# alanqrwang/nwhead

Measured on AMD Instinct MI355X. Metric: query-predictions/sec, higher is better.
Workload: dtype f32; 1 GPU; K3 predict('full'): B=256 queries/step vs bank N=50000 d=512 C=200, bank sharded 1-way, 26 query batches coalesced per launch; B=256, N_support=50000, d=512, C=200, parallelism=support-shard x1

## Files before the change

### nwhead_amd/csrc/fused_f16p12.h

```cpp
#pragma once
#include "fused_f16p.h"

namespace nw {
namespace {

struct P12 : PipeCfg<128, 256, 8, 4, 3> {
    static constexpr int RS = BS / 16, QB = BQP / (16 * NCW);
    static_assert(LDS_BYTES <= 160 * 1024, "LDS of one CU");
};

template <int KIND, bool CAND = false>
__device__ __forceinline__ void epilogue_p12(f32x4 (&acc)[P12::QB][P12::RS], const float* hdr, int nrun, int2 bnd,
                                             float scale, float* __restrict__ ws_m,
                                             float* __restrict__ ws_den, float* __restrict__ ws_num, int B, int N,
                                             int q0, int s0, int st, int wave, int lane, int n_stiles, int k
#ifdef NW_DIAG_FUSED
                                             , unsigned long long (&diag_)[8], unsigned long long& last_
#endif
                                             ) {
    using P = P12;
    constexpr int RS = P::RS, QB = P::QB, BS = P::BS;
    constexpr bool NEED_NORM = (KIND != NW_SCORE_DOT);
    typedef float f32x2 __attribute__((ext_vector_type(2)));
    const float* sn2 = hdr;
    const float* ssc = hdr + P::NH;
    const int* runid = reinterpret_cast<const int*>(hdr + 2 * P::NH);
    const float* qn2 = hdr + 3 * P::NH;
    const float* qsc_s = qn2 + P::BQP;
    const int i = lane & 15, g = lane >> 4;
    using SF = ScoreFactors<KIND>;
    float Cq[QB], Bq[QB];
#pragma unroll
    for (int j = 0; j < QB; ++j) {
        const int qrow = 16 * (QB * wave + j) + i;
        SF::query(NEED_NORM ? qn2[qrow] : 0.f, qsc_s[qrow], scale, Cq[j], Bq[j]);
    }
    NW_PSTAMP(1);
    float sc[QB][RS][4];
#pragma unroll
    for (int r = 0; r < RS; ++r) {
        const float4 n4 = NEED_NORM ? *reinterpret_cast<const float4*>(sn2 + 16 * r + 4 * g) : make_float4(0.f, 0.f, 0.f, 0.f);
        const float4 s4 = *reinterpret_cast<const float4*>(ssc + 16 * r + 4 * g);
        float4 K4, B4;
        SF::support(n4.x, s4.x, K4.x, B4.x);
        SF::support(n4.y, s4.y, K4.y, B4.y);
        SF::support(n4.z, s4.z, K4.z, B4.z);
        SF::support(n4.w, s4.w, K4.w, B4.w);
        float4 B4r = B4;
        asm volatile("" : "+v"(B4r.x), "+v"(B4r.y), "+v"(B4r.z), "+v"(B4r.w));
#pragma unroll
        for (int j = 0; j < QB; ++j) {
            const f32x2 cq = {Cq[j], Cq[j]}, bq = {Bq[j], Bq[j]};
            const float4 Bj = (j == 0) ? B4 : B4r;
            const f32x2 d01 = __builtin_elementwise_fma(f32x2{acc[j][r][0], acc[j][r][1]}, f32x2{K4.x, K4.y} * cq,
                                                        f32x2{Bj.x, Bj.y} + bq);
            const f32x2 d23 = __builtin_elementwise_fma(f32x2{acc[j][r][2], acc[j][r][3]}, f32x2{K4.z, K4.w} * cq,
                                                        f32x2{Bj.z, Bj.w} + bq);
            sc[j][r][0] = SF::finish_abs(d01.x);
            sc[j][r][1] = SF::finish_abs(d01.y);
            sc[j][r][2] = SF::finish_abs(d23.x);
            sc[j][r][3] = SF::finish_abs(d23.y);
            asm volatile("" : "+v"(sc[j][r][0]), "+v"(sc[j][r][1]), "+v"(sc[j][r][2]), "+v"(sc[j][r][3]));
        }
        __builtin_amdgcn_sched_barrier(0);
    }
    NW_PSTAMP(2);
    if constexpr (CAND) {
        int ln = lane;
        asm volatile("" : "+v"(ln));
        const int ci = ln & 15, cg = ln >> 4;
#pragma unroll
        for (int j = 0; j < QB; ++j) {
            float u[RS][4];
#pragma unroll
            for (int r = 0; r < RS; ++r)
#pragma unroll
                for (int e = 0; e < 4; ++e) u[r][e] = SF::DIST ? -sc[j][r][e] : sc[j][r][e];
            tile_candidates<RS>(u, reinterpret_cast<unsigned*>(ws_m), reinterpret_cast<int*>(ws_den), B, N,
                                q0 + 16 * (QB * wave + j) + ci, s0, cg, st, n_stiles, k);
            __builtin_amdgcn_sched_barrier(0);
        }
        return;
    }
    constexpr float WORST = SF::DIST ? INFINITY : -INFINITY;
    if (s0 + BS > N) {
        const int lim = N - s0 - 4 * g;
#pragma unroll
        for (int j = 0; j < QB; ++j)
#pragma unroll
            for (int r = 0; r < RS; ++r)
#pragma unroll
                for (int e = 0; e < 4; ++e)
                    if (16 * r + e >= lim) sc[j][r][e] = WORST;
    }
    auto best = [](float a, float b) { return SF::DIST ? fminf(a, b) : fmaxf(a, b); };
    auto best3 = [&](float a, float b, float c) { return best(best(a, b), c); };
    static_assert(RS == 8, "chain k takes the 16-row blocks k and k + 4");
    float ext[QB];
#pragma unroll
    for (int j = 0; j < QB; ++j) {
        float mx[4];
#pragma unroll
        for (int k = 0; k < 4; ++k) mx[k] = best3(sc[j][k][0], sc[j][k][1], sc[j][k][2]);
#pragma unroll
        for (int k = 0; k < 4; ++k) mx[k] = best3(mx[k], sc[j][k][3], sc[j][k + 4][0]);
#pragma unroll
        for (int k = 0; k < 4; ++k) mx[k] = best3(mx[k], sc[j][k + 4][1], sc[j][k + 4][2]);
#pragma unroll
        for (int k = 0; k < 4; ++k) mx[k] = best(mx[k], sc[j][k + 4][3]);
        ext[j] = best(best3(mx[0], mx[1], mx[2]), mx[3]);
    }
    group4_each(ext, best);
    float mloc[QB], dloc[QB], s0v[QB], s1v[QB] = {0.f, 0.f}, s2v[QB] = {0.f, 0.f};
#pragma unroll
    for (int j = 0; j < QB; ++j) {
        mloc[j] = SF::DIST ? -ext[j] : ext[j];
#pragma unroll
        for (int r = 0; r < RS; ++r)
#pragma unroll
            for (int e = 0; e < 4; ++e)
                sc[j][r][e] = __builtin_amdgcn_exp2f(SF::DIST ? ext[j] - sc[j][r][e] : sc[j][r][e] - ext[j]);
    }
    NW_PSTAMP(3);
    auto add = [](float a, float b) { return a + b; };
    if (nrun <= 3) {
        float S0[QB][2] = {{0.f, 0.f}, {0.f, 0.f}}, S1[QB][2] = {{0.f, 0.f}, {0.f, 0.f}}, S2[QB][2] = {{0.f, 0.f}, {0.f, 0.f}};
        if (nrun == 1) {
#pragma unroll
            for (int r = 0; r < RS; ++r)
#pragma unroll
                for (int j = 0; j < QB; ++j) S0[j][r & 1] += (sc[j][r][0] + sc[j][r][1]) + (sc[j][r][2] + sc[j][r][3]);
        } else {
            const int b1 = bnd.x, b2 = (nrun == 3) ? bnd.y : BS;
            const float L1 = (float)(b1 - 4 * g);
            const float M2 = 1.f - (float)(b2 - 4 * g);
#pragma unroll
            for (int r = 0; r < RS; ++r) {
                const int lo = 16 * r, hi = 16 * r + 16;
                const bool in0 = hi <= b1, in2 = lo >= b2, in1 = lo >= b1 && hi <= b2;
#pragma unroll
                for (int j = 0; j < QB; ++j) {
                    const float quad = (sc[j][r][0] + sc[j][r][1]) + (sc[j][r][2] + sc[j][r][3]);
                    S0[j][r & 1] = __builtin_fmaf(in0 ? 1.f : 0.f, quad, S0[j][r & 1]);
                    S1[j][r & 1] = __builtin_fmaf(in1 ? 1.f : 0.f, quad, S1[j][r & 1]);
                    S2[j][r & 1] = __builtin_fmaf(in2 ? 1.f : 0.f, quad, S2[j][r & 1]);
                }
                if (!(in0 || in1 || in2)) {
#pragma unroll
                    for (int e = 0; e < 4; ++e) {
                        const float c = (float)(16 * r + e);
                        const float w1 = __builtin_amdgcn_fmed3f(L1 - c, 0.f, 1.f);
                        const float u2 = __builtin_amdgcn_fmed3f(c + M2, 0.f, 1.f);
#pragma unroll
                        for (int j = 0; j < QB; ++j) {
                            const float ev = sc[j][r][e];
                            S0[j][e & 1] = __builtin_fmaf(w1, ev, S0[j][e & 1]);
                            S2[j][e & 1] = __builtin_fmaf(u2, ev, S2[j][e & 1]);
                            S1[j][e & 1] = __builtin_fmaf((1.f - w1) - u2, ev, S1[j][e & 1]);
                        }
                    }
                }
            }
        }
        if (nrun == 1) {
            float v[QB] = {S0[0][0] + S0[0][1], S0[1][0] + S0[1][1]};
            group4_each(v, add);
            s0v[0] = v[0], s0v[1] = v[1];
        } else if (nrun == 2) {
            float v[2 * QB] = {S0[0][0] + S0[0][1], S0[1][0] + S0[1][1], S1[0][0] + S1[0][1], S1[1][0] + S1[1][1]};
            group4_each(v, add);
            s0v[0] = v[0], s0v[1] = v[1], s1v[0] = v[2], s1v[1] = v[3];
        } else {
            float v[3 * QB] = {S0[0][0] + S0[0][1], S0[1][0] + S0[1][1], S1[0][0] + S1[0][1],
                               S1[1][0] + S1[1][1], S2[0][0] + S2[0][1], S2[1][0] + S2[1][1]};
            group4_each(v, add);
            s0v[0] = v[0], s0v[1] = v[1], s1v[0] = v[2], s1v[1] = v[3], s2v[0] = v[4], s2v[1] = v[5];
        }
#pragma unroll
        for (int j = 0; j < QB; ++j) dloc[j] = (s0v[j] + s1v[j]) + s2v[j];
    } else {
#pragma unroll
        for (int j = 0; j < QB; ++j) {
            float dl[4] = {0.f, 0.f, 0.f, 0.f};
#pragma unroll
            for (int r = 0; r < RS; ++r) dl[r & 3] += (sc[j][r][0] + sc[j][r][1]) + (sc[j][r][2] + sc[j][r][3]);
            dloc[j] = (dl[0] + dl[1]) + (dl[2] + dl[3]);
        }
        group4_each(dloc, add);
#pragma unroll
        for (int j = 0; j < QB; ++j) {
            const int b = q0 + 16 * (QB * wave + j) + i;
            for (int run_base = 0; run_base < nrun; run_base += 16) {
                f32x4 Pm = {0.f, 0.f, 0.f, 0.f};
                const int want = run_base + i;
#pragma unroll
                for (int r = 0; r < RS; ++r) {
                    const int4 rid = *reinterpret_cast<const int4*>(runid + 16 * r + 4 * g);
                    Pm = __builtin_amdgcn_mfma_f32_16x16x4f32(rid.x == want ? 1.f : 0.f, sc[j][r][0], Pm, 0, 0, 0);
                    Pm = __builtin_amdgcn_mfma_f32_16x16x4f32(rid.y == want ? 1.f : 0.f, sc[j][r][1], Pm, 0, 0, 0);
                    Pm = __builtin_amdgcn_mfma_f32_16x16x4f32(rid.z == want ? 1.f : 0.f, sc[j][r][2], Pm, 0, 0, 0);
                    Pm = __builtin_amdgcn_mfma_f32_16x16x4f32(rid.w == want ? 1.f : 0.f, sc[j][r][3], Pm, 0, 0, 0);
                }
                if (b < B) {
#pragma unroll
                    for (int jj = 0; jj < 4; ++jj) {
                        const int run = run_base + 4 * g + jj;
                        if (run < nrun) ws_num[((size_t)st * BS + run) * B + b] = Pm[jj];
                    }
                }
            }
        }
    }
    NW_PSTAMP(4);
    static_assert(QB == 2, "lane groups 0 / 1 carry query blocks 0 / 1, groups 2 / 3 the same blocks of the next array");
    int ln = lane;
    asm volatile("" : "+v"(ln));
    const int b = q0 + 16 * QB * wave + (ln & 31);
    const bool blk1 = ln & 16, arr1 = ln & 32;
    const size_t tb = (size_t)st * B + b, nb = (size_t)st * BS * B + b;
    if (b < B) {
        const float mv = blk1 ? mloc[1] : mloc[0], dv = blk1 ? dloc[1] : dloc[0];
        (arr1 ? ws_den : ws_m)[tb] = arr1 ? dv : mv;
        if (nrun <= 3) {
            const float n0 = blk1 ? s0v[1] : s0v[0], n1 = blk1 ? s1v[1] : s1v[0], n2 = blk1 ? s2v[1] : s2v[0];
            if (!arr1 || nrun >= 2) ws_num[nb + (arr1 ? B : 0)] = arr1 ? n1 : n0;
            if (!arr1 && nrun == 3) ws_num[nb + 2 * (size_t)B] = n2;
        }
    }
    NW_PSTAMP(5);
}

template <int KIND, bool HALF = false, bool CAND = false>
__global__ __launch_bounds__(P12::THREADS, 3) void nw_fused_f16p_kernel_w12(
    const float* __restrict__ q, const float* __restrict__ s, const float* __restrict__ s_norm2,
    const float* __restrict__ s_scale, const float* __restrict__ q_norm2, const float* __restrict__ q_scale,
    const float* __restrict__ logit_scale, const int* __restrict__ ws_runid, const int* __restrict__ ws_nrun,
    const int* __restrict__ ws_bnd, float* __restrict__ ws_m, float* __restrict__ ws_den, float* __restrict__ ws_num, int B,
    int N, int d, int n_stiles, int n_qtiles, int qg, int k) {
    static_assert(!CAND || HALF, "the candidate form exists for half-precision rows only");
    using P = P12;
    constexpr int RS = P::RS, QB = P::QB, BS = P::BS, BQP = P::BQP, NB = P::NB;
    extern __shared__ __attribute__((aligned(16))) char smem[];
    float* hdr0 = reinterpret_cast<float*>(smem);
    float4* stage = reinterpret_cast<float4*>(smem + P::HDR_BYTES);

    const int tid = threadIdx.x, lane = tid & 63;
    const int wave = __builtin_amdgcn_readfirstlane(tid >> 6);
    const int nk = d / BK;
    const PersistentTiles tiles(blockIdx.x, gridDim.x, n_stiles, n_qtiles, qg);
    const int cu = tiles.cu, n_cu = tiles.n_cu, n_local = tiles.n_local;

    if (wave >= P::NCW) {
        persistent_loader<P, !CAND>(tiles, wave - P::NCW, lane, hdr0, stage, q, s, s_norm2, s_scale, q_norm2, q_scale, ws_runid, B, N,
                             d);
    } else {
        const int i = lane & 15, g = lane >> 4;
        const int rsw = (i >> 1) & 7;
        const int sh = g ^ rsw, sl = (4 + g) ^ rsw;
        const int qoff = (16 * QB * wave + i) * ROW_F4, soff = (BQP + i) * ROW_F4;
        struct QF { float4 bh[QB], bl[QB]; };
        struct SW { float4 al[2], ah[2]; };
        constexpr int NW_ = RS / 2;
        auto rd_q = [&](QF& f, const float4* S) {
#pragma unroll
            for (int j = 0; j < QB; ++j) {
                f.bh[j] = S[qoff + 16 * j * ROW_F4 + sh];
                f.bl[j] = S[qoff + 16 * j * ROW_F4 + sl];
            }
        };
        auto rd_w = [&](SW& w, const float4* S, int p) {
#pragma unroll
            for (int x = 0; x < 2; ++x) {
                w.al[x] = S[soff + 16 * (2 * p + x) * ROW_F4 + sl];
                w.ah[x] = S[soff + 16 * (2 * p + x) * ROW_F4 + sh];
            }
        };
        auto mm = [](const float4& a, const float4& b, f32x4 c) {
            return __builtin_amdgcn_mfma_f32_16x16x32_f16(__builtin_bit_cast(half8, a), __builtin_bit_cast(half8, b), c, 0, 0, 0);
        };
        auto pin = []() { __builtin_amdgcn_sched_barrier(0); };
        f32x4 acc[QB][RS];
        auto mm_w = [&](const SW& w, const QF& f, int p) {
            if constexpr (HALF) {
#pragma unroll
                for (int x = 0; x < 2; ++x)
#pragma unroll
                    for (int j = 0; j < QB; ++j) acc[j][2 * p + x] = mm(w.ah[x], f.bh[j], acc[j][2 * p + x]);
#pragma unroll
                for (int x = 0; x < 2; ++x)
#pragma unroll
                    for (int j = 0; j < QB; ++j) acc[j][2 * p + x] = mm(w.al[x], f.bl[j], acc[j][2 * p + x]);
            } else {
#pragma unroll
                for (int x = 0; x < 2; ++x)
#pragma unroll
                    for (int j = 0; j < QB; ++j) acc[j][2 * p + x] = mm(w.al[x], f.bh[j], acc[j][2 * p + x]);
#pragma unroll
                for (int x = 0; x < 2; ++x)
#pragma unroll
                    for (int j = 0; j < QB; ++j) acc[j][2 * p + x] = mm(w.ah[x], f.bl[j], acc[j][2 * p + x]);
#pragma unroll
                for (int x = 0; x < 2; ++x)
#pragma unroll
                    for (int j = 0; j < QB; ++j) acc[j][2 * p + x] = mm(w.ah[x], f.bh[j], acc[j][2 * p + x]);
            }
            __builtin_amdgcn_sched_barrier(0);
        };
        SW wa, wb;
        auto run_stage = [&](const QF& fp, QF& fc, int slot, auto first) {
            constexpr bool FIRST = decltype(first)::value;
#ifdef NW_ABL_NORD
            constexpr bool RD = FIRST;
#else
            constexpr bool RD = true;
#endif
            const float4* S = stage + slot * P::TILE_F4;
            if (RD) { rd_q(fc, S); rd_w(wa, S, 0); }
            pin();
            if (!FIRST) mm_w(wb, fp, NW_ - 1);
#pragma unroll
            for (int p = 0; p + 1 < NW_; ++p) {
                if (RD) rd_w((p & 1) ? wa : wb, S, p + 1);
                pin();
                mm_w((p & 1) ? wb : wa, fc, p);
            }
            static_assert(NW_ % 2 == 0, "the last pair of a stage sits in wb");
            tile_barrier();
        };
        using Yes = std::integral_constant<bool, true>;
        using No = std::integral_constant<bool, false>;

        float scale = 1.f;
        if (KIND == NW_SCORE_CLIP)
            scale = __builtin_bit_cast(float, __builtin_amdgcn_readfirstlane(__builtin_bit_cast(int, expf(*logit_scale))));
        tile_barrier();
        int gi = 0;
        int par = 0;
        auto next_slot = [&]() {
            const int b = gi;
            gi = (gi + 1 == NB) ? 0 : gi + 1;
            return b;
        };
#ifdef NW_DIAG_FUSED
        unsigned long long diag_[8] = {0, 0, 0, 0, 0, 0, 0, 0}, last_ = __builtin_amdgcn_s_memtime();
        const unsigned long long first_ = last_, first_rt_ = __builtin_amdgcn_s_memrealtime();
#endif
        for (int T = cu; T < n_local; T += n_cu) {
            int qt, st;
            tiles.decode(T, qt, st);
            const int q0 = qt * BQP, s0 = st * BS;
            int nrun = 0;
            int2 bnd = {0, 0};
            if constexpr (!CAND) {
                nrun = ws_nrun[st];
                bnd = *reinterpret_cast<const int2*>(ws_bnd + 2 * (size_t)st);
            }
#pragma unroll
            for (int j = 0; j < QB; ++j)
#pragma unroll
                for (int r = 0; r < RS; ++r) acc[j][r] = f32x4{0.f, 0.f, 0.f, 0.f};
            QF f0, f1;
#ifdef NW_ABL_NORD
            rd_q(f1, stage + gi * P::TILE_F4);
#endif
            run_stage(f1, f0, next_slot(), Yes{});
            int kt = 1;
            for (; kt + 1 < nk; kt += 2) {
                run_stage(f0, f1, next_slot(), No{});
                run_stage(f1, f0, next_slot(), No{});
            }
            if (kt < nk) {
                run_stage(f0, f1, next_slot(), No{});
                mm_w(wb, f1, NW_ - 1);
            } else {
                mm_w(wb, f0, NW_ - 1);
            }
            NW_PSTAMP(0);
#ifndef NW_ABL_NOEPI
            epilogue_p12<KIND, CAND>(acc, hdr0 + par * P::HDR_F, nrun, bnd, scale, ws_m, ws_den, ws_num, B, N, q0, s0, st, wave,
                                     lane, n_stiles, k
#ifdef NW_DIAG_FUSED
                                     , diag_, last_
#endif
                                     );
#else
            keep_acc_alive(acc, ws_m, nrun, bnd);
#endif
            par = (par + 1 == P::NHB) ? 0 : par + 1;
            NW_PSTAMP(6);
        }
#ifdef NW_DIAG_FUSED
        diag_write_out(diag_, last_, first_, first_rt_);
#endif
    }
}

}
}
```

Before: 7.653 million query-predictions/s.

## Interleave LDS fragment reads with individual MFMAs and use incrementing LDS pointers

Replaces the grouped read-then-MFMA pattern in the compute waves with a per-MFMA schedule. Each LDS read for the next query and support fragments is issued between single MFMA instructions, separated by sched_barrier pins, so that LDS latency hides behind matrix work, including across the stage boundary. LDS addresses are now kept as raw address-space-3 offsets that advance per ring slot, instead of being recomputed from the slot index. It also adds optional head-timing diagnostics, and the rigid manual schedule may lose to the compiler's own scheduling or raise register pressure.

```diff
diff --git a/nwhead_amd/csrc/fused_f16p12.h b/nwhead_amd/csrc/fused_f16p12.h
--- a/nwhead_amd/csrc/fused_f16p12.h
+++ b/nwhead_amd/csrc/fused_f16p12.h
@@ -261,52 +261,70 @@
         struct QF { float4 bh[QB], bl[QB]; };
         struct SW { float4 al[2], ah[2]; };
         constexpr int NW_ = RS / 2;
-        auto rd_q = [&](QF& f, const float4* S) {
-#pragma unroll
-            for (int j = 0; j < QB; ++j) {
-                f.bh[j] = S[qoff + 16 * j * ROW_F4 + sh];
-                f.bl[j] = S[qoff + 16 * j * ROW_F4 + sl];
-            }
-        };
-        auto rd_w = [&](SW& w, const float4* S, int p) {
-#pragma unroll
-            for (int x = 0; x < 2; ++x) {
-                w.al[x] = S[soff + 16 * (2 * p + x) * ROW_F4 + sl];
-                w.ah[x] = S[soff + 16 * (2 * p + x) * ROW_F4 + sh];
-            }
-        };
+#ifdef NW_DIAG_FUSED
+        unsigned long long diag_[8] = {0, 0, 0, 0, 0, 0, 0, 0}, last_ = 0;
+#endif
+#ifdef NW_DIAG_HEAD
+        unsigned long long h0_ = 0, h1_ = 0;
+#define NW_HEAD_STAMP(t) asm volatile("s_memtime %0" : "=s"(t))
+#else
+#define NW_HEAD_STAMP(t)
+#endif
         auto mm = [](const float4& a, const float4& b, f32x4 c) {
             return __builtin_amdgcn_mfma_f32_16x16x32_f16(__builtin_bit_cast(half8, a), __builtin_bit_cast(half8, b), c, 0, 0, 0);
         };
         auto pin = []() { __builtin_amdgcn_sched_barrier(0); };
         f32x4 acc[QB][RS];
-        auto mm_w = [&](const SW& w, const QF& f, int p) {
-            if constexpr (HALF) {
-#pragma unroll
-                for (int x = 0; x < 2; ++x)
-#pragma unroll
-                    for (int j = 0; j < QB; ++j) acc[j][2 * p + x] = mm(w.ah[x], f.bh[j], acc[j][2 * p + x]);
-#pragma unroll
-                for (int x = 0; x < 2; ++x)
-#pragma unroll
-                    for (int j = 0; j < QB; ++j) acc[j][2 * p + x] = mm(w.al[x], f.bl[j], acc[j][2 * p + x]);
+        constexpr int NM = HALF ? 8 : 12;
+        auto mm_1 = [&](const SW& w, const QF& f, int p, int m) {
+            const int ph = m >> 2, x = (m >> 1) & 1, j = m & 1;
+            const float4& a = HALF ? (ph == 0 ? w.ah[x] : w.al[x]) : (ph == 0 ? w.al[x] : w.ah[x]);
+            const float4& b = HALF ? (ph == 0 ? f.bh[j] : f.bl[j]) : (ph == 1 ? f.bl[j] : f.bh[j]);
+            acc[j][2 * p + x] = mm(a, b, acc[j][2 * p + x]);
+        };
+        auto mm_w = [&](const SW& w, const QF& f, int p, auto&& behind) {
+#pragma unroll
+            for (int m = 0; m < NM; ++m) {
+                mm_1(w, f, p, m);
+                behind(m);
+            }
+            pin();
+        };
+        auto nothing = [](int) {};
+        typedef const __attribute__((address_space(3))) f32x4 lds_f4;
+        const unsigned ring0 = (unsigned)(uintptr_t)(__attribute__((address_space(3))) char*)(char*)stage;
+        unsigned a_qh = ring0 + 16u * (qoff + sh), a_ql = ring0 + 16u * (qoff + sl);
+        unsigned a_sh = ring0 + 16u * (soff + sh), a_sl = ring0 + 16u * (soff + sl);
+        asm volatile("" : "+v"(a_qh), "+v"(a_ql), "+v"(a_sh), "+v"(a_sl));
+        auto lds_rd = [](unsigned a, int f4) { return __builtin_bit_cast(float4, *(lds_f4*)(uintptr_t)(a + 16u * f4)); };
+        auto q_h = [&](int j) { return lds_rd(a_qh, 16 * j * ROW_F4); };
+        auto q_l = [&](int j) { return lds_rd(a_ql, 16 * j * ROW_F4); };
+        auto s_h = [&](int blk) { return lds_rd(a_sh, 16 * blk * ROW_F4); };
+        auto s_l = [&](int blk) { return lds_rd(a_sl, 16 * blk * ROW_F4); };
+        auto advance = [&](int slot, int m) {
+            const unsigned step = (slot + 1 == NB) ? 0u - (unsigned)((NB - 1) * P::TILE_F4 * 16) : (unsigned)(P::TILE_F4 * 16);
+            unsigned& a = (m == 0) ? a_qh : (m == 1) ? a_ql : (m == 2) ? a_sh : a_sl;
+            a += step;
+            asm volatile("" : "+v"(a));
+        };
+        SW wa, wb;
+        auto rd_first = [&](QF& f, SW& w, int n) {
+            const bool qlo = n >= 4, slo = (n < 4) != HALF;
+            const int r = n & 3;
+            if (r == 0 || r == 3) {
+                const int x = r == 3;
+                if (slo) w.al[x] = s_l(x);
+                else w.ah[x] = s_h(x);
             } else {
-#pragma unroll
-                for (int x = 0; x < 2; ++x)
-#pragma unroll
-                    for (int j = 0; j < QB; ++j) acc[j][2 * p + x] = mm(w.al[x], f.bh[j], acc[j][2 * p + x]);
-#pragma unroll
-                for (int x = 0; x < 2; ++x)
-#pragma unroll
-                    for (int j = 0; j < QB; ++j) acc[j][2 * p + x] = mm(w.ah[x], f.bl[j], acc[j][2 * p + x]);
-#pragma unroll
-                for (int x = 0; x < 2; ++x)
-#pragma unroll
-                    for (int j = 0; j < QB; ++j) acc[j][2 * p + x] = mm(w.ah[x], f.bh[j], acc[j][2 * p + x]);
-            }
-            __builtin_amdgcn_sched_barrier(0);
-        };
-        SW wa, wb;
+                if (qlo) f.bl[r - 1] = q_l(r - 1);
+                else f.bh[r - 1] = q_h(r - 1);
+            }
+        };
+        auto rd_pair = [&](SW& w, int p, int n) {
+            const int x = n & 1;
+            if ((n < 2) != HALF) w.al[x] = s_l(2 * p + x);
+            else w.ah[x] = s_h(2 * p + x);
+        };
         auto run_stage = [&](const QF& fp, QF& fc, int slot, auto first) {
             constexpr bool FIRST = decltype(first)::value;
 #ifdef NW_ABL_NORD
@@ -314,18 +332,43 @@
 #else
             constexpr bool RD = true;
 #endif
-            const float4* S = stage + slot * P::TILE_F4;
-            if (RD) { rd_q(fc, S); rd_w(wa, S, 0); }
-            pin();
-            if (!FIRST) mm_w(wb, fp, NW_ - 1);
+            if constexpr (FIRST) {
+#pragma unroll
+                for (int n = 0; n < 8; ++n) {
+                    rd_first(fc, wa, n);
+                    pin();
+                }
+            } else {
+                NW_HEAD_STAMP(h0_);
+                mm_w(wb, fp, NW_ - 1, [&](int m) {
+                    if (m == 0) NW_HEAD_STAMP(h1_);
+                    if (m < 8) {
+                        pin();
+                        if (RD) rd_first(fc, wa, m);
+                        pin();
+                    }
+                });
+            }
 #pragma unroll
             for (int p = 0; p + 1 < NW_; ++p) {
-                if (RD) rd_w((p & 1) ? wa : wb, S, p + 1);
-                pin();
-                mm_w((p & 1) ? wb : wa, fc, p);
+                SW& wr = (p & 1) ? wa : wb;
+                mm_w((p & 1) ? wb : wa, fc, p, [&](int m) {
+                    if (m < 4) {
+                        pin();
+                        if (RD) rd_pair(wr, p + 1, m);
+                        pin();
+                    } else if (p + 2 == NW_ && m < 8) {
+                        pin();
+                        advance(slot, m - 4);
+                        pin();
+                    }
+                });
             }
             static_assert(NW_ % 2 == 0, "the last pair of a stage sits in wb");
             tile_barrier();
+#ifdef NW_DIAG_HEAD
+            if (!FIRST) diag_[6] += h1_ - h0_;
+#endif
         };
         using Yes = std::integral_constant<bool, true>;
         using No = std::integral_constant<bool, false>;
@@ -342,7 +385,7 @@
             return b;
         };
 #ifdef NW_DIAG_FUSED
-        unsigned long long diag_[8] = {0, 0, 0, 0, 0, 0, 0, 0}, last_ = __builtin_amdgcn_s_memtime();
+        last_ = __builtin_amdgcn_s_memtime();
         const unsigned long long first_ = last_, first_rt_ = __builtin_amdgcn_s_memrealtime();
 #endif
         for (int T = cu; T < n_local; T += n_cu) {
@@ -361,7 +404,8 @@
                 for (int r = 0; r < RS; ++r) acc[j][r] = f32x4{0.f, 0.f, 0.f, 0.f};
             QF f0, f1;
 #ifdef NW_ABL_NORD
-            rd_q(f1, stage + gi * P::TILE_F4);
+#pragma unroll
+            for (int n = 0; n < 8; ++n) rd_first(f1, wa, n);
 #endif
             run_stage(f1, f0, next_slot(), Yes{});
             int kt = 1;
@@ -371,9 +415,9 @@
             }
             if (kt < nk) {
                 run_stage(f0, f1, next_slot(), No{});
-                mm_w(wb, f1, NW_ - 1);
+                mm_w(wb, f1, NW_ - 1, nothing);
             } else {
-                mm_w(wb, f0, NW_ - 1);
+                mm_w(wb, f0, NW_ - 1, nothing);
             }
             NW_PSTAMP(0);
 #ifndef NW_ABL_NOEPI
@@ -387,7 +431,9 @@
             keep_acc_alive(acc, ws_m, nrun, bnd);
 #endif
             par = (par + 1 == P::NHB) ? 0 : par + 1;
+#ifndef NW_DIAG_HEAD
             NW_PSTAMP(6);
+#endif
         }
 #ifdef NW_DIAG_FUSED
         diag_write_out(diag_, last_, first_, first_rt_);
```

New measurement: 7.854 million query-predictions/s, median of 6. 1.03x the previous value.
